# Medical-Image-Analysis-Laboratory/MSLesions3D

Hardware: AMD Instinct MI355X
Metric: training volumes/sec at 128^3 batch-4 (fwd+loss+bwd+Adam), data-parallel over N MI355X (higher is better)
Workload: dtype f32; 1 GPU; 128^3 synthetic volumes, batch 4/GPU, 1 channel(s), fp32, SSD3D+MobileNet3D full train step (BASELINE configs[1]); global_batch=4, parallelism=dp1, priors=9344

## Files before the change

### mslesions3d_amd/csrc/pwconv.hip

```cpp
#include "common.hpp"
#include <algorithm>
#include <cstdlib>

namespace {

typedef float f32x16 __attribute__((ext_vector_type(16)));

constexpr int BM = 64, BN = 128, BK = 32;
constexpr int FOLD_MAXK = 512;
constexpr int WS_LD = BK + 1;

template <bool AFFINE, bool STATS, bool TRANS_W>
__global__ __launch_bounds__(256) void pw_gemm_kernel(const float* __restrict__ X,
                                                      const float* __restrict__ in_scale,
                                                      const float* __restrict__ in_shift,
                                                      const float* __restrict__ Wt, float* __restrict__ Y,
                                                      double* __restrict__ partials, int M, int K, int S,
                                                      msl::BnFold fold) {
  __shared__ __align__(16) float Xs[BK][BN];
  __shared__ float Ws[BM][WS_LD];
  __shared__ float red[2][2][BM];
  __shared__ float f_sc[AFFINE ? FOLD_MAXK : 1], f_sh[AFFINE ? FOLD_MAXK : 1];
  const int n = blockIdx.z, m0 = blockIdx.y * BM, s0 = blockIdx.x * BN;
  const int tid = threadIdx.x, lane = tid & 63, wv = tid >> 6;
// ... 571 lines not shown
                     0, st, X, in_scale, in_shift, Wt, Y, partials, M, K, S, fold)
#define MSL_WV1(KW_, MT_)                                                                                              \
  do {                                                                                                                 \
    if (nt == 2)                                                                                                       \
      MSL_LAUNCH((pw_wave_kernel<KW_, MT_, AFFINE, STATS, TRANS_W, 1, 2>), dim3(msl::cdiv(S, 256), M / (32 * MT_), N), \
                         dim3(256), 0, st, X, in_scale, in_shift, Wt, Y, partials, M, K, S, fold);                     \
    else                                                                                                               \
      MSL_WV(KW_, MT_, 1);                                                                                             \
  } while (0)
  const bool two = M % 64 == 0;
  const int nt = STATS ? wave_nt(N, K, M, S) : 1;
  if (K == 32) {
    if (two) MSL_WV1(32, 2); else MSL_WV1(32, 1);
  } else if (K == 64) {
    if (two) MSL_WV1(64, 2); else MSL_WV1(64, 1);
  } else {
    switch (K / 64) {
      case 2: MSL_WV(64, 1, 2); break;
      case 4: MSL_WV(64, 1, 4); break;
      case 8: MSL_WV(64, 1, 8); break;
      default: return MSL_ERR_UNSUPPORTED;
    }
  }
#undef MSL_WV1
#undef MSL_WV
  MSL_LAUNCH_CHECK();
  return MSL_OK;
}

constexpr int PC = 64, PC_LD = PC + 1;

template <int BNN, bool AFFINE>
__global__ __launch_bounds__(256) void pw_bwd_weight_kernel(const float* __restrict__ dY,
                                                            const float* __restrict__ Z,
                                                            const float* __restrict__ in_scale,
                                                            const float* __restrict__ in_shift,
                                                            float* __restrict__ slabs, int Cout, int Cin,
                                                            int S, int N, int chunks_per_img,
                                                            int chunks_per_block) {
  constexpr int NSUB_N = BNN / 32;
  constexpr int NSUB = 2 * NSUB_N;
  __shared__ __align__(16) float lds[(64 + BNN) * PC_LD > 64 * BNN ? (64 + BNN) * PC_LD : 64 * BNN];
  float* dys = lds;
  float* as_ = lds + 64 * PC_LD;
  const int ks = blockIdx.x;
  const int tiles_n = Cin / BNN;
  const int tm = blockIdx.y / tiles_n, tn = blockIdx.y % tiles_n;
  const int m0 = tm * 64, n0 = tn * BNN;
  const int tid = threadIdx.x, lane = tid & 63, wv = tid >> 6;
  const int total_chunks = N * chunks_per_img;
  const int ch_lo = ks * chunks_per_block, ch_hi = min(total_chunks, ch_lo + chunks_per_block);
  const bool vec_ok = (S & 3) == 0;

  f32x16 acc[NSUB];
#pragma unroll
  for (int i = 0; i < NSUB; ++i) acc[i] = (f32x16){0};

  float scv[BNN / 16], shv[BNN / 16];
#pragma unroll
  for (int j = 0; j < BNN / 16; ++j) {
    scv[j] = AFFINE ? in_scale[n0 + (tid >> 4) + j * 16] : 1.f;
    shv[j] = AFFINE ? in_shift[n0 + (tid >> 4) + j * 16] : 0.f;
  }

  for (int ch = ch_lo; ch < ch_hi; ++ch) {
    const int n = ch / chunks_per_img, s0 = (ch % chunks_per_img) * PC;
    const float* dyn = dY + ((size_t)n * Cout + m0) * S;
    const float* zn = Z + ((size_t)n * Cin + n0) * S;
    float4 st[(64 + BNN) / 16];
    if (vec_ok) {
#pragma unroll
      for (int i = 0; i < (64 + BNN) / 16; ++i) {
        const int r = (tid >> 4) + i * 16;
        st[i] = msl::load4_zfill<true>(r < 64 ? dyn + (size_t)r * S : zn + (size_t)(r - 64) * S, s0 + (tid & 15) * 4, S);
      }
    } else {
#pragma unroll
      for (int i = 0; i < (64 + BNN) / 16; ++i) {
        const int r = (tid >> 4) + i * 16;
        st[i] = msl::load4_zfill<false>(r < 64 ? dyn + (size_t)r * S : zn + (size_t)(r - 64) * S, s0 + (tid & 15) * 4, S);
      }
    }
#pragma unroll
    for (int i = 0; i < (64 + BNN) / 16; ++i) {
      const int r = (tid >> 4) + i * 16, c4 = (tid & 15) * 4, col = s0 + c4;
      float4 v = st[i];
      if (AFFINE && r >= 64) {
        const float sc = scv[i >= 4 ? i - 4 : 0], sh = shv[i >= 4 ? i - 4 : 0];
        v.x = col < S ? msl::act(v.x, sc, sh) : 0.f;
        v.y = col + 1 < S ? msl::act(v.y, sc, sh) : 0.f;
        v.z = col + 2 < S ? msl::act(v.z, sc, sh) : 0.f;
        v.w = col + 3 < S ? msl::act(v.w, sc, sh) : 0.f;
      }
      float* dst = lds + r * PC_LD + c4;
      dst[0] = v.x; dst[1] = v.y; dst[2] = v.z; dst[3] = v.w;
    }
    __syncthreads();
#pragma unroll
    for (int kk = 0; kk < 8; ++kk) {
      const int pos = wv * 16 + 2 * kk + (lane >> 5);
      float a[2], b[NSUB_N];
#pragma unroll
      for (int i = 0; i < 2; ++i) a[i] = dys[(i * 32 + (lane & 31)) * PC_LD + pos];
#pragma unroll
      for (int j = 0; j < NSUB_N; ++j) b[j] = as_[(j * 32 + (lane & 31)) * PC_LD + pos];
#pragma unroll
      for (int i = 0; i < 2; ++i)
#pragma unroll
        for (int j = 0; j < NSUB_N; ++j)
          acc[i * NSUB_N + j] = __builtin_amdgcn_mfma_f32_32x32x2f32(a[i], b[j], acc[i * NSUB_N + j], 0, 0, 0);
    }
    __syncthreads();
  }

  float* redt = lds;
  for (int w = 3; w >= 1; --w) {
    if (wv == w) {
#pragma unroll
      for (int i = 0; i < 2; ++i)
#pragma unroll
        for (int j = 0; j < NSUB_N; ++j)
#pragma unroll
          for (int r = 0; r < 16; ++r) {
            const int row = i * 32 + (r & 3) + 8 * (r >> 2) + 4 * (lane >> 5);
            const int col = j * 32 + (lane & 31);
            const float v = acc[i * NSUB_N + j][r];
            if (w == 3) redt[row * BNN + col] = v;
            else redt[row * BNN + col] += v;
          }
    }
    __syncthreads();
  }
  if (wv == 0) {
    float* out = slabs + (size_t)ks * Cout * Cin;
#pragma unroll
    for (int i = 0; i < 2; ++i)
#pragma unroll
      for (int j = 0; j < NSUB_N; ++j)
#pragma unroll
        for (int r = 0; r < 16; ++r) {
          const int row = i * 32 + (r & 3) + 8 * (r >> 2) + 4 * (lane >> 5);
          const int col = j * 32 + (lane & 31);
          out[(size_t)(m0 + row) * Cin + n0 + col] = acc[i * NSUB_N + j][r] + redt[row * BNN + col];
        }
  }
}

template <int MT, bool AFFINE>
__device__ __forceinline__ void pw_bww_wave_body(const float* __restrict__ dY, const float* __restrict__ Z,
                                                 const float* __restrict__ in_scale, const float* __restrict__ in_shift,
                                                 float* __restrict__ out, int Cout, int Cin, int S, int chunks_per_img,
                                                 int total_chunks, int chunks_per_block, int ks, int tile) {
  __shared__ __align__(16) float red[4 * MT * 1024];
  const int lane = threadIdx.x & 63, wv = threadIdx.x >> 6, h = lane >> 5, c = lane & 31;
  const int tiles_n = Cin / 32;
  const int tm = tile / tiles_n, tn = tile % tiles_n;
  const int m0 = tm * 32 * MT, n0 = tn * 32;
  const int ch_lo = ks * chunks_per_block, ch_hi = min(total_chunks, ch_lo + chunks_per_block);
  const int mine = max(0, (ch_hi - ch_lo - wv + 3) / 4);

  float sc = 1.f, sh = 0.f;
  if (AFFINE) {
    sc = in_scale[n0 + c];
    sh = in_shift[n0 + c];
  }
  f32x16 acc[MT];
#pragma unroll
  for (int mt = 0; mt < MT; ++mt) acc[mt] = (f32x16){0};

  float4 a0[MT][4], b0[4], a1[MT][4], b1[4];
  auto issue = [&](int i, float4 (&a)[MT][4], float4 (&b)[4]) {
    const int ch = min(ch_lo + wv + 4 * i, total_chunks - 1);
    const int n = ch / chunks_per_img, s0 = (ch - n * chunks_per_img) * 32 + 16 * h;
#pragma unroll
    for (int mt = 0; mt < MT; ++mt) {
      const float4* p = reinterpret_cast<const float4*>(dY + ((size_t)n * Cout + m0 + mt * 32 + c) * S + s0);
#pragma unroll
      for (int j = 0; j < 4; ++j) a[mt][j] = p[j];
    }
    const float4* q = reinterpret_cast<const float4*>(Z + ((size_t)n * Cin + n0 + c) * S + s0);
#pragma unroll
    for (int j = 0; j < 4; ++j) b[j] = q[j];
  };
  auto mac = [&](float4 (&a)[MT][4], float4 (&b)[4]) {
#pragma unroll
    for (int j = 0; j < 4; ++j) {
      float bv[4] = {b[j].x, b[j].y, b[j].z, b[j].w};
#pragma unroll
      for (int e = 0; e < 4; ++e) {
        const float x = AFFINE ? msl::act(bv[e], sc, sh) : bv[e];
#pragma unroll
        for (int mt = 0; mt < MT; ++mt) {
          const float av = e == 0 ? a[mt][j].x : e == 1 ? a[mt][j].y : e == 2 ? a[mt][j].z : a[mt][j].w;
          acc[mt] = __builtin_amdgcn_mfma_f32_32x32x2f32(av, x, acc[mt], 0, 0, 0);
        }
      }
    }
  };

  if (mine > 0) issue(0, a0, b0);
#pragma unroll 1
  for (int i = 0; i < mine; i += 2) {
    issue(i + 1, a1, b1);
    __builtin_amdgcn_sched_barrier(0);
    mac(a0, b0);
    if (i + 1 < mine) {
      issue(i + 2, a0, b0);
      __builtin_amdgcn_sched_barrier(0);
      mac(a1, b1);
    }
  }

#pragma unroll
  for (int mt = 0; mt < MT; ++mt)
#pragma unroll
    for (int r = 0; r < 16; ++r) red[((wv * MT + mt) * 32 + (r & 3) + 8 * (r >> 2) + 4 * h) * 32 + c] = acc[mt][r];
  __syncthreads();
  float* dst = out + (size_t)ks * Cout * Cin;
#pragma unroll
  for (int e = 0; e < MT; ++e) {
    const int q4 = threadIdx.x + e * 256;
    const int row = q4 >> 3, col = (q4 & 7) * 4;
    float4 v = *reinterpret_cast<const float4*>(&red[(0 * MT * 32 + row) * 32 + col]);
#pragma unroll
    for (int w2 = 1; w2 < 4; ++w2) {
      const float4 t = *reinterpret_cast<const float4*>(&red[(w2 * MT * 32 + row) * 32 + col]);
      v.x += t.x; v.y += t.y; v.z += t.z; v.w += t.w;
    }
    *reinterpret_cast<float4*>(dst + (size_t)(m0 + row) * Cin + n0 + col) = v;
  }
}

template <int MT, bool AFFINE>
__global__ __launch_bounds__(256) void pw_bww_wave_kernel(const float* __restrict__ dY, const float* __restrict__ Z,
                                                          const float* __restrict__ in_scale,
                                                          const float* __restrict__ in_shift, float* __restrict__ out,
                                                          int Cout, int Cin, int S, int chunks_per_img, int total_chunks,
                                                          int chunks_per_block) {
  pw_bww_wave_body<MT, AFFINE>(dY, Z, in_scale, in_shift, out, Cout, Cin, S, chunks_per_img, total_chunks, chunks_per_block,
                               blockIdx.x, blockIdx.y);
}

constexpr int PW_BWW_BATCH_MAX = 4;
struct PwBwwBatch {
  const float* dY[PW_BWW_BATCH_MAX];
  const float* Z[PW_BWW_BATCH_MAX];
  const float* in_scale[PW_BWW_BATCH_MAX];
  const float* in_shift[PW_BWW_BATCH_MAX];
  float* out[PW_BWW_BATCH_MAX];
  int Cout[PW_BWW_BATCH_MAX], Cin[PW_BWW_BATCH_MAX], S[PW_BWW_BATCH_MAX], chunks_per_img[PW_BWW_BATCH_MAX],
      total_chunks[PW_BWW_BATCH_MAX], chunks_per_block[PW_BWW_BATCH_MAX], ksplit[PW_BWW_BATCH_MAX],
      first[PW_BWW_BATCH_MAX + 1];
};

__global__ __launch_bounds__(256) void pw_bww_wave_batch_kernel(PwBwwBatch b, int n) {
  int k = 0;
#pragma unroll
  for (int j = 1; j < PW_BWW_BATCH_MAX; ++j)
    if (j < n && (int)blockIdx.x >= b.first[j]) k = j;
  const int local = blockIdx.x - b.first[k];
  pw_bww_wave_body<2, true>(b.dY[k], b.Z[k], b.in_scale[k], b.in_shift[k], b.out[k], b.Cout[k], b.Cin[k], b.S[k],
                            b.chunks_per_img[k], b.total_chunks[k], b.chunks_per_block[k], local % b.ksplit[k],
                            local / b.ksplit[k]);
}

struct BwwWavePlan {
  int mt, tiles, chunks_per_img, total_chunks, ksplit, chunks_per_block;
};

static inline bool bww_wave_plan(int N, int Cin, int Cout, int S, BwwWavePlan& p) {
  constexpr int off = 1;
  if (!off || S % 32 != 0 || Cin % 32 != 0 || Cout % 32 != 0) return false;
  p.mt = (Cout % 64 == 0) ? 2 : 1;
  p.tiles = (Cout / (32 * p.mt)) * (Cin / 32);
  p.chunks_per_img = S / 32;
  p.total_chunks = N * p.chunks_per_img;
  constexpr int target = 256;
  int ks = std::max(1, std::min(target / std::max(1, p.tiles), p.total_chunks / 8));
  p.chunks_per_block = msl::cdiv(p.total_chunks, ks);
  p.ksplit = msl::cdiv(p.total_chunks, p.chunks_per_block);
  return true;
}

__global__ __launch_bounds__(256) void slab_reduce_kernel(const float* __restrict__ slabs, float* __restrict__ out,
                                                          int count, int nslabs) {
  __shared__ float lds[8 * 33];
  const float t = msl::reduce_slabs_256(slabs, (size_t)count, count, nslabs, lds);
  const int i = blockIdx.x * 32 + (threadIdx.x & 31);
  if ((threadIdx.x >> 5) == 0 && i < count) out[i] = t;
}

struct BwPlan {
  int bnn, ksplit, chunks_per_img, chunks_per_block;
};

BwPlan bw_plan(int N, int Cin, int Cout, int S) {
  BwPlan p;
  p.bnn = (Cin % 64 == 0) ? 64 : 32;
  p.chunks_per_img = msl::cdiv(S, PC);
  const int total = N * p.chunks_per_img;
  const int tiles = (Cout / 64) * (Cin / p.bnn);
  int ks = std::max(1, std::min(total, 512 / std::max(1, tiles)));
  constexpr int min_cpb = 1;
  ks = std::max(1, std::min(ks, total / std::max(1, min_cpb)));
  p.chunks_per_block = msl::cdiv(total, ks);
  p.ksplit = msl::cdiv(total, p.chunks_per_block);
  return p;
}

}

extern "C" {

static inline bool use_ksplit(int K, int M, int S, int N) {
  return K >= 128 && K % 128 == 0 && msl::cdiv(S, BN) * msl::cdiv(M, BM) * N < 256;
}

int msl_pwconv_fwd_num_partials(int N, int Cin, int Cout, int S) {
  if (const int cols = strip_cols(N, Cin, Cout, S)) return N * (S / cols);
  if (wave_form(Cin, Cout)) return N * msl::cdiv(S, Cin <= 64 ? 128 * wave_nt(N, Cin, Cout, S) : 32);
  return N * msl::cdiv(S, use_ksplit(Cin, Cout, S, N) ? KS_BN : BN);
}

static const msl::BnFold pw_nofold{nullptr, 0, 0, 1.0, nullptr, nullptr, 0.f};

static int pwconv_fwd_impl(const float* z, const float* in_scale, const float* in_shift, const msl::BnFold& fold,
                           const float* w, float* y, double* partials, int N, int Cin, int Cout, int S, void* stream) {
  if (N <= 0 || S <= 0 || Cin % BK != 0 || Cout % 4 != 0) return MSL_ERR_ARG;
  if ((in_scale || fold.partials) && Cin > FOLD_MAXK) return MSL_ERR_UNSUPPORTED;
  hipStream_t st = (hipStream_t)stream;
  if (const int cols = strip_cols(N, Cin, Cout, S)) {
    if (in_scale || fold.partials) {
      if (partials) return launch_strip<true, true, false>(z, in_scale, in_shift, w, y, partials, N, Cout, Cin, S, cols, fold, st);
      return launch_strip<true, false, false>(z, in_scale, in_shift, w, y, partials, N, Cout, Cin, S, cols, fold, st);
    }
    if (partials) return launch_strip<false, true, false>(z, in_scale, in_shift, w, y, partials, N, Cout, Cin, S, cols, fold, st);
    return launch_strip<false, false, false>(z, in_scale, in_shift, w, y, partials, N, Cout, Cin, S, cols, fold, st);
  }
  if (wave_form(Cin, Cout)) {
    if (in_scale || fold.partials) {
      if (partials) return launch_wave<true, true, false>(z, in_scale, in_shift, w, y, partials, N, Cout, Cin, S, fold, st);
      return launch_wave<true, false, false>(z, in_scale, in_shift, w, y, partials, N, Cout, Cin, S, fold, st);
    }
    if (partials) return launch_wave<false, true, false>(z, in_scale, in_shift, w, y, partials, N, Cout, Cin, S, fold, st);
    return launch_wave<false, false, false>(z, in_scale, in_shift, w, y, partials, N, Cout, Cin, S, fold, st);
  }
  if (use_ksplit(Cin, Cout, S, N)) {
    dim3 g2(msl::cdiv(S, KS_BN), msl::cdiv(Cout, KS_BM), N);
#define MSL_KS(A_, S_, T_, X_, Wp_, Y_, P_, M_, K_)                                                                  \
  do {                                                                                                             \
    if ((K_) % 256 == 0) {                                                                                         \
      const size_t lds_ = (size_t)8 * KS_WAVE_LDS * sizeof(float);                                                 \
      hipError_t e_ = hipFuncSetAttribute(reinterpret_cast<const void*>(pw_gemm_ksplit_kernel<A_, S_, T_, 8>),    \
                                          hipFuncAttributeMaxDynamicSharedMemorySize, (int)lds_);                  \
      if (e_ != hipSuccess) return (int)e_;                                                                        \
      MSL_LAUNCH((pw_gemm_ksplit_kernel<A_, S_, T_, 8>), g2, dim3(512), lds_, st, X_, in_scale, in_shift,  \
                         Wp_, Y_, P_, M_, K_, S, fold);                                                            \
    } else {                                                                                                       \
      MSL_LAUNCH((pw_gemm_ksplit_kernel<A_, S_, T_, 4>), g2, dim3(256),                                    \
                         (size_t)4 * KS_WAVE_LDS * sizeof(float), st, X_, in_scale, in_shift, Wp_, Y_, P_, M_, K_, S, fold); \
    }                                                                                                              \
  } while (0)
    if (in_scale || fold.partials) {
      if (partials) MSL_KS(true, true, false, z, w, y, partials, Cout, Cin);
      else MSL_KS(true, false, false, z, w, y, partials, Cout, Cin);
    } else {
      if (partials) MSL_KS(false, true, false, z, w, y, partials, Cout, Cin);
      else MSL_KS(false, false, false, z, w, y, partials, Cout, Cin);
    }
    MSL_LAUNCH_CHECK();
    return MSL_OK;
  }
  dim3 grid(msl::cdiv(S, BN), msl::cdiv(Cout, BM), N);
  if (in_scale || fold.partials) {
    if (partials) MSL_LAUNCH((pw_gemm_kernel<true, true, false>), grid, dim3(256), 0, st, z, in_scale, in_shift, w, y, partials, Cout, Cin, S, fold);
    else MSL_LAUNCH((pw_gemm_kernel<true, false, false>), grid, dim3(256), 0, st, z, in_scale, in_shift, w, y, partials, Cout, Cin, S, fold);
  } else {
    if (partials) MSL_LAUNCH((pw_gemm_kernel<false, true, false>), grid, dim3(256), 0, st, z, in_scale, in_shift, w, y, partials, Cout, Cin, S, fold);
    else MSL_LAUNCH((pw_gemm_kernel<false, false, false>), grid, dim3(256), 0, st, z, in_scale, in_shift, w, y, partials, Cout, Cin, S, fold);
  }
  MSL_LAUNCH_CHECK();
  return MSL_OK;
}

int msl_pwconv_fwd(const float* z, const float* in_scale, const float* in_shift, const float* w, float* y,
                   double* partials, int N, int Cin, int Cout, int S, void* stream) {
  return pwconv_fwd_impl(z, in_scale, in_shift, pw_nofold, w, y, partials, N, Cin, Cout, S, stream);
}

int msl_pwconv_fwd_fold(const float* z, const double* in_partials, int in_np, double in_count, const float* gamma,
                        const float* beta, float eps, const float* w, float* y, double* partials, int N, int Cin,
                        int Cout, int S, void* stream) {
  if (!in_partials || in_np <= 0) return MSL_ERR_ARG;
  const msl::BnFold fold{in_partials, in_np, Cin, in_count, gamma, beta, eps};
  return pwconv_fwd_impl(z, nullptr, nullptr, fold, w, y, partials, N, Cin, Cout, S, stream);
}

int msl_pwconv_bwd_data(const float* dy, const float* w, float* g_in, int N, int Cin, int Cout, int S,
                        void* stream) {
  if (N <= 0 || S <= 0 || Cout % BK != 0 || Cin % 4 != 0) return MSL_ERR_ARG;
  if (const int cols = strip_cols(N, Cout, Cin, S))
    return launch_strip<false, false, true>(dy, nullptr, nullptr, w, g_in, nullptr, N, Cin, Cout, S, cols, pw_nofold,
                                            (hipStream_t)stream);
  if (wave_form(Cout, Cin))
    return launch_wave<false, false, true>(dy, nullptr, nullptr, w, g_in, nullptr, N, Cin, Cout, S, pw_nofold,
                                           (hipStream_t)stream);
  if (use_ksplit(Cout, Cin, S, N)) {
    dim3 g2(msl::cdiv(S, KS_BN), msl::cdiv(Cin, KS_BM), N);
    hipStream_t st = (hipStream_t)stream;
    const float *in_scale = nullptr, *in_shift = nullptr;
    double* nopart = nullptr;
    const msl::BnFold fold = pw_nofold;
    MSL_KS(false, false, true, dy, w, g_in, nopart, Cin, Cout);
    MSL_LAUNCH_CHECK();
    return MSL_OK;
  }
  dim3 grid(msl::cdiv(S, BN), msl::cdiv(Cin, BM), N);
  MSL_LAUNCH((pw_gemm_kernel<false, false, true>), grid, dim3(256), 0, (hipStream_t)stream, dy, nullptr,
                     nullptr, w, g_in, nullptr, Cin, Cout, S, pw_nofold);
  MSL_LAUNCH_CHECK();
  return MSL_OK;
}

size_t msl_pwconv_bwd_weight_workspace_bytes(int N, int Cin, int Cout, int S) {
  BwwWavePlan wp;
  if (bww_wave_plan(N, Cin, Cout, S, wp)) return (size_t)wp.ksplit * Cout * Cin * sizeof(float);
  BwPlan p = bw_plan(N, Cin, Cout, S);
  return (size_t)p.ksplit * Cout * Cin * sizeof(float);
}

int msl_pwconv_bwd_weight_nslabs(int N, int Cin, int Cout, int S) {
// ... 85 lines not shown
```

### mslesions3d_amd/csrc/chanlink.hip

```cpp
#include "common.hpp"
#include "../../include/mslesions3d_hip.h"

namespace {

typedef float f32x4v __attribute__((ext_vector_type(4)));

template <typename T>
__device__ __forceinline__ f32x4v ldq(const T* p) {
  const float4 v = msl::ld4(p);
  return (f32x4v){v.x, v.y, v.z, v.w};
}
template <typename T>
__device__ __forceinline__ void stq(T* p, f32x4v v) { msl::st4(p, make_float4(v[0], v[1], v[2], v[3])); }
template <typename T>
__device__ __forceinline__ f32x4v rounded(const T* tag, f32x4v v) {
  const float4 r = msl::as_stored(tag, make_float4(v[0], v[1], v[2], v[3]));
  return (f32x4v){r.x, r.y, r.z, r.w};
}

template <int NW>
__device__ __forceinline__ void chan_sum2(double& a, double& b, double* scratch) {
  a = msl::wave_sum(a);
  b = msl::wave_sum(b);
  if (NW > 1) {
    const int lane = threadIdx.x & 63, w = threadIdx.x >> 6;
    __syncthreads();
    if (lane == 0) {
      scratch[2 * w] = a;
      scratch[2 * w + 1] = b;
    }
    __syncthreads();
    a = 0.0;
    b = 0.0;
#pragma unroll
    for (int i = 0; i < NW; ++i) {
      a += scratch[2 * i];
      b += scratch[2 * i + 1];
    }
  }
}

template <typename T, int NW, int QO, int QI, int STRIDE, bool BWW>
__global__ __launch_bounds__(NW * 64) void block_bwd_channel_link_kernel(
    T* __restrict__ g_z, const T* __restrict__ z, const float* __restrict__ vec_z, const float* __restrict__ w_dw,
    const T* __restrict__ y_prev, const float* __restrict__ vec_y, T* __restrict__ g_y,
    float* __restrict__ dgamma_z, float* __restrict__ dbeta_z, float* __restrict__ dgamma_y, float* __restrict__ dbeta_y,
    float* __restrict__ dw_dw, int N, int C, int lD, int lH, int lW, int accumulate) {
  constexpr int NT = NW * 64, LS = STRIDE == 2 ? 1 : 0;
  extern __shared__ __align__(16) float lds[];
  const int c = blockIdx.x, tid = threadIdx.x;
  const int lOD = lD - LS, lOH = lH - LS, lOW = lW - LS;
  const int OD = 1 << lOD, OH = 1 << lOH, OW = 1 << lOW;
  const int lSo = lOD + lOH + lOW, lSi = lD + lH + lW;
  const int tot_qo = N << (lSo - 2), tot_qi = N << (lSi - 2);
  const int PW = OW + 8, PP = (OH + 2) * PW, pimg = (OD + 2) * PP, ptot = N * pimg;
  double* scratch = reinterpret_cast<double*>(lds + (BWW ? max(ptot, 27 * NT + 27 * 4) : ptot));

  f32x4v gq[QO], zq[QO], yq[QI], aq[QI];
#pragma unroll
  for (int q = 0; q < QO; ++q) {
    const int qi = min(tid + q * NT, tot_qo - 1), n = qi >> (lSo - 2), r = qi & ((1 << (lSo - 2)) - 1);
    const size_t off = (((size_t)n * C + c) << lSo) + 4 * r;
    gq[q] = ldq(g_z + off);
    zq[q] = ldq(z + off);
  }
#pragma unroll
  for (int q = 0; q < QI; ++q) {
    const int qi = min(tid + q * NT, tot_qi - 1), n = qi >> (lSi - 2), r = qi & ((1 << (lSi - 2)) - 1);
    yq[q] = ldq(y_prev + (((size_t)n * C + c) << lSi) + 4 * r);
  }
  if (accumulate) {
#pragma unroll
    for (int q = 0; q < QI; ++q) {
      const int qi = min(tid + q * NT, tot_qi - 1), n = qi >> (lSi - 2), r = qi & ((1 << (lSi - 2)) - 1);
      aq[q] = ldq(g_y + (((size_t)n * C + c) << lSi) + 4 * r);
    }
  } else {
#pragma unroll
    for (int q = 0; q < QI; ++q) aq[q] = (f32x4v){0.f, 0.f, 0.f, 0.f};
  }
  const float sc1 = vec_z[c], sh1 = vec_z[C + c], mu1 = vec_z[2 * C + c], is1 = vec_z[3 * C + c];
  const float sc2 = vec_y[c], sh2 = vec_y[C + c], mu2 = vec_y[2 * C + c], is2 = vec_y[3 * C + c];
  float wt[27];
#pragma unroll
  for (int k = 0; k < 27; ++k) wt[k] = w_dw[c * 27 + k];
  for (int i = tid; i < (ptot >> 2); i += NT) reinterpret_cast<f32x4v*>(lds)[i] = (f32x4v){0.f, 0.f, 0.f, 0.f};

  float s1 = 0.f, s2 = 0.f;
#pragma unroll
  for (int q = 0; q < QO; ++q) {
    const bool in = tid + q * NT < tot_qo;
#pragma unroll
    for (int e = 0; e < 4; ++e) {
      const float gm = (in && fmaf(zq[q][e], sc1, sh1) > 0.f) ? gq[q][e] : 0.f;
      const float xh = (zq[q][e] - mu1) * is1;
      gq[q][e] = gm;
      zq[q][e] = xh;
      s1 += gm;
      s2 += gm * xh;
    }
  }
  double t1 = (double)s1, t2 = (double)s2;
  chan_sum2<NW>(t1, t2, scratch);
  {
    const double cnt_o = (double)(N << lSo);
    const float k1 = (float)(t1 / cnt_o), k2 = (float)(t2 / cnt_o);
    if (tid == 0) {
      dbeta_z[c] = (float)t1;
      dgamma_z[c] = (float)t2;
    }
    if (NW == 1) __syncthreads();
#pragma unroll
    for (int q = 0; q < QO; ++q) {
      const int qi = tid + q * NT;
      if (qi < tot_qo) {
        const int n = qi >> (lSo - 2), r = qi & ((1 << (lSo - 2)) - 1);
        f32x4v dz;
#pragma unroll
        for (int e = 0; e < 4; ++e) dz[e] = sc1 * (gq[q][e] - k1 - zq[q][e] * k2);
        stq(g_z + (((size_t)n * C + c) << lSo) + 4 * r, dz);
        dz = rounded(g_z, dz);
        const int s = 4 * r, ow = s & (OW - 1), oh = (s >> lOW) & (OH - 1), od = s >> (lOW + lOH);
        *reinterpret_cast<f32x4v*>(lds + n * pimg + (od + 1) * PP + (oh + 1) * PW + 4 + ow) = dz;
      }
    }
  }
  __syncthreads();

  s1 = 0.f;
  s2 = 0.f;
  const int W = 1 << lW, H = 1 << lH;
  float dwa[BWW ? 27 : 1];
#pragma unroll
  for (int k = 0; k < (BWW ? 27 : 1); ++k) dwa[k] = 0.f;
#pragma unroll
  for (int q = 0; q < QI; ++q) {
    const int qi = tid + q * NT;
    const bool in = qi < tot_qi;
    const int qc = in ? qi : 0, n = qc >> (lSi - 2), r = qc & ((1 << (lSi - 2)) - 1);
    const int s = 4 * r, iw = s & (W - 1), ih = (s >> lW) & (H - 1), id = s >> (lW + lH);
    f32x4v acc = aq[q];
    f32x4v av;
#pragma unroll
    for (int e = 0; e < 4; ++e) av[e] = (BWW && in) ? msl::act(yq[q][e], sc2, sh2) : 0.f;
    const float* img = lds + n * pimg + 4;
#pragma unroll
    for (int kd = 0; kd < 3; ++kd) {
      const int td = id + 1 - kd;
      if (STRIDE == 2 && (td & 1)) continue;
      const int pd = (STRIDE == 2 ? (td >> 1) : td) + 1;
#pragma unroll
      for (int kh = 0; kh < 3; ++kh) {
        const int th = ih + 1 - kh;
        if (STRIDE == 2 && (th & 1)) continue;
        const int ph = (STRIDE == 2 ? (th >> 1) : th) + 1;
        const float* row = img + pd * PP + ph * PW;
        const float w0 = wt[kd * 9 + kh * 3], w1 = wt[kd * 9 + kh * 3 + 1], w2 = wt[kd * 9 + kh * 3 + 2];
        if (STRIDE == 1) {
          const float lft = row[iw - 1], rgt = row[iw + 4];
          const f32x4v m = *reinterpret_cast<const f32x4v*>(row + iw);
          acc[0] = fmaf(w0, m[1], fmaf(w1, m[0], fmaf(w2, lft, acc[0])));
          acc[1] = fmaf(w0, m[2], fmaf(w1, m[1], fmaf(w2, m[0], acc[1])));
          acc[2] = fmaf(w0, m[3], fmaf(w1, m[2], fmaf(w2, m[1], acc[2])));
          acc[3] = fmaf(w0, rgt, fmaf(w1, m[3], fmaf(w2, m[2], acc[3])));
          if (BWW) {
            float& d0 = dwa[kd * 9 + kh * 3];
            float& d1 = dwa[kd * 9 + kh * 3 + 1];
            float& d2 = dwa[kd * 9 + kh * 3 + 2];
            d0 = fmaf(av[0], m[1], fmaf(av[1], m[2], fmaf(av[2], m[3], fmaf(av[3], rgt, d0))));
            d1 = fmaf(av[0], m[0], fmaf(av[1], m[1], fmaf(av[2], m[2], fmaf(av[3], m[3], d1))));
            d2 = fmaf(av[0], lft, fmaf(av[1], m[0], fmaf(av[2], m[1], fmaf(av[3], m[2], d2))));
          }
        } else {
          const int o = iw >> 1;
          const float2 r01 = *reinterpret_cast<const float2*>(row + o);
          const float r2 = row[o + 2];
          acc[0] = fmaf(w1, r01.x, acc[0]);
          acc[1] = fmaf(w0, r01.y, fmaf(w2, r01.x, acc[1]));
          acc[2] = fmaf(w1, r01.y, acc[2]);
          acc[3] = fmaf(w0, r2, fmaf(w2, r01.y, acc[3]));
          if (BWW) {
            float& d0 = dwa[kd * 9 + kh * 3];
            float& d1 = dwa[kd * 9 + kh * 3 + 1];
            float& d2 = dwa[kd * 9 + kh * 3 + 2];
            d0 = fmaf(av[1], r01.y, fmaf(av[3], r2, d0));
            d1 = fmaf(av[0], r01.x, fmaf(av[2], r01.y, d1));
            d2 = fmaf(av[1], r01.x, fmaf(av[3], r01.y, d2));
          }
        }
      }
    }
    acc = rounded(g_y, acc);
#pragma unroll
    for (int e = 0; e < 4; ++e) {
      const float gm = (in && fmaf(yq[q][e], sc2, sh2) > 0.f) ? acc[e] : 0.f;
      const float xh = (yq[q][e] - mu2) * is2;
      aq[q][e] = gm;
      yq[q][e] = xh;
      s1 += gm;
      s2 += gm * xh;
    }
  }
  if (BWW) {
    __syncthreads();
#pragma unroll
    for (int k = 0; k < 27; ++k) lds[k * NT + tid] = dwa[k];
    __syncthreads();
    constexpr int PART = NT / 4;
    for (int t = tid; t < 108; t += NT) {
      const int k = t >> 2, part = t & 3;
      const f32x4v* src = reinterpret_cast<const f32x4v*>(lds + k * NT + part * PART);
      double sum = 0.0;
#pragma unroll 4
      for (int i = 0; i < PART / 4; ++i) {
        const f32x4v v = src[i];
        sum += (double)v[0];
        sum += (double)v[1];
        sum += (double)v[2];
        sum += (double)v[3];
      }
      sum += msl::dpp_mov<0xB1>(sum);
      sum += msl::dpp_mov<0x4E>(sum);
      if (part == 0) dw_dw[c * 27 + k] = (float)sum;
    }
  }
  t1 = (double)s1;
  t2 = (double)s2;
  chan_sum2<NW>(t1, t2, scratch);
  const double cnt_i = (double)(N << lSi);
  const float k1 = (float)(t1 / cnt_i), k2 = (float)(t2 / cnt_i);
  if (tid == 0) {
    dbeta_y[c] = (float)t1;
    dgamma_y[c] = (float)t2;
  }
#pragma unroll
  for (int q = 0; q < QI; ++q) {
    const int qi = tid + q * NT;
    if (qi < tot_qi) {
      const int n = qi >> (lSi - 2), r = qi & ((1 << (lSi - 2)) - 1);
      f32x4v dy;
#pragma unroll
      for (int e = 0; e < 4; ++e) dy[e] = sc2 * (aq[q][e] - k1 - yq[q][e] * k2);
      stq(g_y + (((size_t)n * C + c) << lSi) + 4 * r, dy);
    }
  }
}

struct LinkPlan {
  int nw, qo, qi, lD, lH, lW;
  size_t smem;
};

static inline int ilog2_exact(int v) {
  int l = 0;
  while ((1 << l) < v) ++l;
  return (1 << l) == v ? l : -1;
}

bool link_plan(int N, int D, int H, int W, int stride, LinkPlan& p) {
  if (N <= 0 || D <= 0 || H <= 0 || W <= 0 || (stride != 1 && stride != 2)) return false;
  p.lD = ilog2_exact(D);
  p.lH = ilog2_exact(H);
  p.lW = ilog2_exact(W);
  if (p.lD < 0 || p.lH < 0 || p.lW < 2) return false;
  const int OD = (D - 1) / stride + 1, OH = (H - 1) / stride + 1, OW = (W - 1) / stride + 1;
  if (OW < 4 || (stride == 2 && (D < 2 || H < 2))) return false;
  const long long tqo = (long long)N * OD * OH * OW / 4, tqi = (long long)N * D * H * W / 4;
  if (tqi <= 128) p.nw = 1;
  else if (tqi <= 1024) p.nw = 4;
  else if (tqi <= 2048) p.nw = 8;
  else if (tqi <= 4096) p.nw = 16;
  else return false;
  const int nt = p.nw * 64;
  auto up = [](long long v) { return v <= 1 ? 1 : v <= 2 ? 2 : 4; };
  p.qi = up((tqi + nt - 1) / nt);
  p.qo = up((tqo + nt - 1) / nt);
  if (p.qo > 1) p.qo = p.qi;
  const size_t ptot = (size_t)N * (OD + 2) * (OH + 2) * (OW + 8);
  p.smem = std::max(ptot, (size_t)27 * nt + 27 * 4) * 4 + 2 * p.nw * sizeof(double);
  return p.smem <= 156 * 1024;
}

}

extern "C" int msl_block_bwd_channel_link_supported(int N, int D, int H, int W, int stride) {
  LinkPlan p;
  return link_plan(N, D, H, W, stride, p) ? p.nw : 0;
}

template <typename T>
static int link_launch(T* g_z, const T* z, const float* vec_z, const float* w_dw, const T* y_prev, const float* vec_y, T* g_y,
                       float* dgamma_z, float* dbeta_z, float* dgamma_y, float* dbeta_y, float* dw_dw, int N, int C, int D,
                       int H, int W, int stride, int accumulate, void* stream) {
  if (N <= 0 || C <= 0 || !g_z || !z || !vec_z || !w_dw || !y_prev || !vec_y || !g_y) return MSL_ERR_ARG;
  LinkPlan p;
  if (!link_plan(N, D, H, W, stride, p)) return MSL_ERR_UNSUPPORTED;
  hipStream_t st = (hipStream_t)stream;
#define MSL_LINK_B(NW_, QO_, QI_, S_, B_)                                                                                 \
  do {                                                                                                                   \
    auto k = block_bwd_channel_link_kernel<T, NW_, QO_, QI_, S_, B_>;                                                    \
    if (p.smem > 64 * 1024) (void)hipFuncSetAttribute((const void*)k, hipFuncAttributeMaxDynamicSharedMemorySize, (int)p.smem); \
    MSL_LAUNCH(k, dim3(C), dim3(NW_ * 64), p.smem, st, g_z, z, vec_z, w_dw, y_prev, vec_y, g_y, dgamma_z, dbeta_z, \
                       dgamma_y, dbeta_y, dw_dw, N, C, p.lD, p.lH, p.lW, accumulate);                                     \
  } while (0)
#define MSL_LINK_S(NW_, QO_, QI_, S_)                  \
  do {                                                 \
    if (dw_dw) MSL_LINK_B(NW_, QO_, QI_, S_, true);    \
    else MSL_LINK_B(NW_, QO_, QI_, S_, false);         \
  } while (0)
#define MSL_LINK_Q(NW_, S_)                                            \
  do {                                                                 \
    if (p.qi == 1) MSL_LINK_S(NW_, 1, 1, S_);                          \
    else if (p.qi == 2 && p.qo == 1) MSL_LINK_S(NW_, 1, 2, S_);        \
    else if (p.qi == 2) MSL_LINK_S(NW_, 2, 2, S_);                     \
    else if (p.qo == 1) MSL_LINK_S(NW_, 1, 4, S_);                     \
    else MSL_LINK_S(NW_, 4, 4, S_);                                    \
  } while (0)
#define MSL_LINK(NW_)                       \
  do {                                      \
    if (stride == 1) MSL_LINK_Q(NW_, 1);    \
    else MSL_LINK_Q(NW_, 2);                \
  } while (0)
  if (p.nw == 1) MSL_LINK(1);
  else if (p.nw == 4) MSL_LINK(4);
  else if (p.nw == 8) MSL_LINK(8);
  else MSL_LINK(16);
#undef MSL_LINK
#undef MSL_LINK_Q
#undef MSL_LINK_S
#undef MSL_LINK_B
  MSL_LAUNCH_CHECK();
  return MSL_OK;
}

extern "C" {

int msl_block_bwd_channel_link(float* g_z, const float* z, const float* vec_z, const float* w_dw, const float* y_prev,
                               const float* vec_y, float* g_y, float* dgamma_z, float* dbeta_z, float* dgamma_y,
                               float* dbeta_y, float* dw_dw, int N, int C, int D, int H, int W, int stride, int accumulate,
                               void* stream) {
  return link_launch<float>(g_z, z, vec_z, w_dw, y_prev, vec_y, g_y, dgamma_z, dbeta_z, dgamma_y, dbeta_y, dw_dw, N, C, D, H, W,
                            stride, accumulate, stream);
}

int msl_block_bwd_channel_link_bf16(void* g_z, const void* z, const float* vec_z, const float* w_dw, const void* y_prev,
                                    const float* vec_y, void* g_y, float* dgamma_z, float* dbeta_z, float* dgamma_y,
                                    float* dbeta_y, float* dw_dw, int N, int C, int D, int H, int W, int stride, int accumulate,
                                    void* stream) {
  return link_launch<msl::su16>((msl::su16*)g_z, (const msl::su16*)z, vec_z, w_dw, (const msl::su16*)y_prev, vec_y,
                                (msl::su16*)g_y, dgamma_z, dbeta_z, dgamma_y, dbeta_y, dw_dw, N, C, D, H, W, stride, accumulate,
                                stream);
}

}
```

Measured before the change: 6062 volumes/s.

## Issue all chunk loads up front for short wave loops and deepen k-split

In the weight-gradient wave kernel, when a wave owns at most four chunks, all dY and Z loads are now issued before any MFMA work. A compile-time-unrolled path handles these cases, so more loads are in flight at once than with the old two-stage ping-pong. The split heuristic now allows a deeper k-split (at least 4 chunks per block instead of 8), falling back to the old floor when the tile grid is small. The wave index is made scalar with readfirstlane. Costs are higher register pressure from four staged buffers and more partial slabs to reduce afterwards.

```diff
diff --git a/mslesions3d_amd/csrc/pwconv.hip b/mslesions3d_amd/csrc/pwconv.hip
--- a/mslesions3d_amd/csrc/pwconv.hip
+++ b/mslesions3d_amd/csrc/pwconv.hip
@@ -747,7 +747,8 @@
                                                  float* __restrict__ out, int Cout, int Cin, int S, int chunks_per_img,
                                                  int total_chunks, int chunks_per_block, int ks, int tile) {
   __shared__ __align__(16) float red[4 * MT * 1024];
-  const int lane = threadIdx.x & 63, wv = threadIdx.x >> 6, h = lane >> 5, c = lane & 31;
+  const int lane = threadIdx.x & 63, h = lane >> 5, c = lane & 31;
+  const int wv = __builtin_amdgcn_readfirstlane(threadIdx.x >> 6);
   const int tiles_n = Cin / 32;
   const int tm = tile / tiles_n, tn = tile % tiles_n;
   const int m0 = tm * 32 * MT, n0 = tn * 32;
@@ -763,7 +764,7 @@
 #pragma unroll
   for (int mt = 0; mt < MT; ++mt) acc[mt] = (f32x16){0};
 
-  float4 a0[MT][4], b0[4], a1[MT][4], b1[4];
+  float4 a[4][MT][4], b[4][4];
   auto issue = [&](int i, float4 (&a)[MT][4], float4 (&b)[4]) {
     const int ch = min(ch_lo + wv + 4 * i, total_chunks - 1);
     const int n = ch / chunks_per_img, s0 = (ch - n * chunks_per_img) * 32 + 16 * h;
@@ -793,16 +794,34 @@
     }
   };
 
-  if (mine > 0) issue(0, a0, b0);
+  if (mine <= 4) {
+    auto walk = [&](auto count) {
+      constexpr int NC = decltype(count)::value;
+#pragma unroll
+      for (int i = 0; i < NC; ++i) issue(i, a[i], b[i]);
+      __builtin_amdgcn_sched_barrier(0);
+#pragma unroll
+      for (int i = 0; i < NC; ++i) mac(a[i], b[i]);
+    };
+    switch (mine) {
+      case 1: walk(std::integral_constant<int, 1>{}); break;
+      case 2: walk(std::integral_constant<int, 2>{}); break;
+      case 3: walk(std::integral_constant<int, 3>{}); break;
+      case 4: walk(std::integral_constant<int, 4>{}); break;
+      default: break;
+    }
+  } else {
+    issue(0, a[0], b[0]);
 #pragma unroll 1
-  for (int i = 0; i < mine; i += 2) {
-    issue(i + 1, a1, b1);
-    __builtin_amdgcn_sched_barrier(0);
-    mac(a0, b0);
-    if (i + 1 < mine) {
-      issue(i + 2, a0, b0);
+    for (int i = 0; i < mine; i += 2) {
+      issue(i + 1, a[1], b[1]);
       __builtin_amdgcn_sched_barrier(0);
-      mac(a1, b1);
+      mac(a[0], b[0]);
+      if (i + 1 < mine) {
+        issue(i + 2, a[0], b[0]);
+        __builtin_amdgcn_sched_barrier(0);
+        mac(a[1], b[1]);
+      }
     }
   }
 
@@ -871,7 +890,9 @@
   p.chunks_per_img = S / 32;
   p.total_chunks = N * p.chunks_per_img;
   constexpr int target = 256;
-  int ks = std::max(1, std::min(target / std::max(1, p.tiles), p.total_chunks / 8));
+  auto split = [&](int floor) { return std::max(1, std::min(target / std::max(1, p.tiles), p.total_chunks / floor)); };
+  int ks = split(4);
+  if (p.tiles * ks < target / 2) ks = split(8);
   p.chunks_per_block = msl::cdiv(p.total_chunks, ks);
   p.ksplit = msl::cdiv(p.total_chunks, p.chunks_per_block);
   return true;
```

After: 6082 volumes/s, median of 5. About the same (+0.3%).

## Assign stride-2 channel-link input quads to threads by spatial parity class

Applied to the files above, without the earlier changes.

For the stride-2 transposed depthwise backward, input quads are now mapped to threads so that every wave shares one (depth, height) parity class, chosen wave-uniformly via readfirstlane. Each wave then runs only the 1, 2 or 4 kernel rows that contribute for its parity, with no per-tap parity branches and no divergence. This is meant to cut the branching and wasted work inside the unrolled 3x3 tap loop. In exchange it adds static constraints on NW/QI, forces QI=4 when NW=1 at stride 2, narrows the set of supported launch configurations (others now return unsupported), and reorders global loads and stores, which may hurt coalescing.

```diff
diff --git a/mslesions3d_amd/csrc/chanlink.hip b/mslesions3d_amd/csrc/chanlink.hip
--- a/mslesions3d_amd/csrc/chanlink.hip
+++ b/mslesions3d_amd/csrc/chanlink.hip
@@ -38,6 +38,35 @@
       b += scratch[2 * i + 1];
     }
   }
+}
+
+constexpr int ilog2c(int v) { return v <= 1 ? 0 : 1 + ilog2c(v >> 1); }
+
+template <int NW, int QI>
+__device__ __forceinline__ int link_parity_class(int q, int tid) {
+  constexpr int LNT = ilog2c(NW * 64);
+  static_assert(QI == 4 || (QI == 2 && NW >= 2) || (QI == 1 && NW >= 4), "the class bits must lie above the lane bits");
+  if (QI == 4) return q;
+  if (QI == 2) return 2 * q + __builtin_amdgcn_readfirstlane(tid >> (LNT - 1));
+  return __builtin_amdgcn_readfirstlane(tid >> (LNT - 2));
+}
+
+template <bool BWW, int KD, int KH>
+__device__ __forceinline__ f32x4v link_row_s2(const float* row, const float* wt, f32x4v av, f32x4v acc, float* dwa) {
+  constexpr int K = KD * 9 + KH * 3;
+  const float w0 = wt[K], w1 = wt[K + 1], w2 = wt[K + 2];
+  const float2 r01 = *reinterpret_cast<const float2*>(row);
+  const float r2 = row[2];
+  acc[0] = fmaf(w1, r01.x, acc[0]);
+  acc[1] = fmaf(w0, r01.y, fmaf(w2, r01.x, acc[1]));
+  acc[2] = fmaf(w1, r01.y, acc[2]);
+  acc[3] = fmaf(w0, r2, fmaf(w2, r01.y, acc[3]));
+  if (BWW) {
+    dwa[K] = fmaf(av[1], r01.y, fmaf(av[3], r2, dwa[K]));
+    dwa[K + 1] = fmaf(av[0], r01.x, fmaf(av[2], r01.y, dwa[K + 1]));
+    dwa[K + 2] = fmaf(av[1], r01.x, fmaf(av[3], r01.y, dwa[K + 2]));
+  }
+  return acc;
 }
 
 template <typename T, int NW, int QO, int QI, int STRIDE, bool BWW>
@@ -56,6 +85,24 @@
   const int PW = OW + 8, PP = (OH + 2) * PW, pimg = (OD + 2) * PP, ptot = N * pimg;
   double* scratch = reinterpret_cast<double*>(lds + (BWW ? max(ptot, 27 * NT + 27 * 4) : ptot));
 
+  auto in_quad = [&](int q, int& n, int& r) -> bool {
+    if constexpr (STRIDE == 1) {
+      const int qi = tid + q * NT, qc = min(qi, tot_qi - 1);
+      n = qc >> (lSi - 2);
+      r = qc & ((1 << (lSi - 2)) - 1);
+      return qi < tot_qi;
+    } else {
+      const int cls = link_parity_class<NW, QI>(q, tid), pa = cls >> 1, pb = (cls ^ pa) & 1;
+      const int rest = tid & ((NT * QI >> 2) - 1);
+      const int x = rest & ((1 << (lSi - 4)) - 1), nn = rest >> (lSi - 4);
+      const int iwq = x & ((1 << (lW - 2)) - 1), ih = ((x >> (lW - 2)) & ((1 << (lH - 1)) - 1)) * 2 + pb;
+      const int id = (x >> (lW + lH - 3)) * 2 + pa;
+      n = min(nn, N - 1);
+      r = (((id << lH) + ih) << (lW - 2)) + iwq;
+      return nn < N;
+    }
+  };
+
   f32x4v gq[QO], zq[QO], yq[QI], aq[QI];
 #pragma unroll
   for (int q = 0; q < QO; ++q) {
@@ -66,13 +113,15 @@
   }
 #pragma unroll
   for (int q = 0; q < QI; ++q) {
-    const int qi = min(tid + q * NT, tot_qi - 1), n = qi >> (lSi - 2), r = qi & ((1 << (lSi - 2)) - 1);
+    int n, r;
+    in_quad(q, n, r);
     yq[q] = ldq(y_prev + (((size_t)n * C + c) << lSi) + 4 * r);
   }
   if (accumulate) {
 #pragma unroll
     for (int q = 0; q < QI; ++q) {
-      const int qi = min(tid + q * NT, tot_qi - 1), n = qi >> (lSi - 2), r = qi & ((1 << (lSi - 2)) - 1);
+      int n, r;
+      in_quad(q, n, r);
       aq[q] = ldq(g_y + (((size_t)n * C + c) << lSi) + 4 * r);
     }
   } else {
@@ -129,34 +178,29 @@
 
   s1 = 0.f;
   s2 = 0.f;
-  const int W = 1 << lW, H = 1 << lH;
   float dwa[BWW ? 27 : 1];
 #pragma unroll
   for (int k = 0; k < (BWW ? 27 : 1); ++k) dwa[k] = 0.f;
 #pragma unroll
   for (int q = 0; q < QI; ++q) {
-    const int qi = tid + q * NT;
-    const bool in = qi < tot_qi;
-    const int qc = in ? qi : 0, n = qc >> (lSi - 2), r = qc & ((1 << (lSi - 2)) - 1);
-    const int s = 4 * r, iw = s & (W - 1), ih = (s >> lW) & (H - 1), id = s >> (lW + lH);
+    int n, r;
+    const bool in = in_quad(q, n, r);
+    const int iwq = r & ((1 << (lW - 2)) - 1), ih = (r >> (lW - 2)) & ((1 << lH) - 1), id = r >> (lW + lH - 2);
     f32x4v acc = aq[q];
     f32x4v av;
 #pragma unroll
     for (int e = 0; e < 4; ++e) av[e] = (BWW && in) ? msl::act(yq[q][e], sc2, sh2) : 0.f;
     const float* img = lds + n * pimg + 4;
-#pragma unroll
-    for (int kd = 0; kd < 3; ++kd) {
-      const int td = id + 1 - kd;
-      if (STRIDE == 2 && (td & 1)) continue;
-      const int pd = (STRIDE == 2 ? (td >> 1) : td) + 1;
-#pragma unroll
-      for (int kh = 0; kh < 3; ++kh) {
-        const int th = ih + 1 - kh;
-        if (STRIDE == 2 && (th & 1)) continue;
-        const int ph = (STRIDE == 2 ? (th >> 1) : th) + 1;
-        const float* row = img + pd * PP + ph * PW;
-        const float w0 = wt[kd * 9 + kh * 3], w1 = wt[kd * 9 + kh * 3 + 1], w2 = wt[kd * 9 + kh * 3 + 2];
-        if (STRIDE == 1) {
+    if constexpr (STRIDE == 1) {
+      const int iw = 4 * iwq;
+#pragma unroll
+      for (int kd = 0; kd < 3; ++kd) {
+        const int pd = id + 2 - kd;
+#pragma unroll
+        for (int kh = 0; kh < 3; ++kh) {
+          const int ph = ih + 2 - kh;
+          const float* row = img + pd * PP + ph * PW;
+          const float w0 = wt[kd * 9 + kh * 3], w1 = wt[kd * 9 + kh * 3 + 1], w2 = wt[kd * 9 + kh * 3 + 2];
           const float lft = row[iw - 1], rgt = row[iw + 4];
           const f32x4v m = *reinterpret_cast<const f32x4v*>(row + iw);
           acc[0] = fmaf(w0, m[1], fmaf(w1, m[0], fmaf(w2, lft, acc[0])));
@@ -171,23 +215,24 @@
             d1 = fmaf(av[0], m[0], fmaf(av[1], m[1], fmaf(av[2], m[2], fmaf(av[3], m[3], d1))));
             d2 = fmaf(av[0], lft, fmaf(av[1], m[0], fmaf(av[2], m[1], fmaf(av[3], m[2], d2))));
           }
-        } else {
-          const int o = iw >> 1;
-          const float2 r01 = *reinterpret_cast<const float2*>(row + o);
-          const float r2 = row[o + 2];
-          acc[0] = fmaf(w1, r01.x, acc[0]);
-          acc[1] = fmaf(w0, r01.y, fmaf(w2, r01.x, acc[1]));
-          acc[2] = fmaf(w1, r01.y, acc[2]);
-          acc[3] = fmaf(w0, r2, fmaf(w2, r01.y, acc[3]));
-          if (BWW) {
-            float& d0 = dwa[kd * 9 + kh * 3];
-            float& d1 = dwa[kd * 9 + kh * 3 + 1];
-            float& d2 = dwa[kd * 9 + kh * 3 + 2];
-            d0 = fmaf(av[1], r01.y, fmaf(av[3], r2, d0));
-            d1 = fmaf(av[0], r01.x, fmaf(av[2], r01.y, d1));
-            d2 = fmaf(av[1], r01.x, fmaf(av[3], r01.y, d2));
-          }
         }
+      }
+    } else {
+      const int cls = link_parity_class<NW, QI>(q, tid), pa = cls >> 1, pb = (cls ^ pa) & 1;
+      const float* row = img + ((id >> 1) + 1) * PP + ((ih >> 1) + 1) * PW + 2 * iwq;
+      if (pa == 0 && pb == 0) {
+        acc = link_row_s2<BWW, 1, 1>(row, wt, av, acc, dwa);
+      } else if (pa == 0) {
+        acc = link_row_s2<BWW, 1, 0>(row + PW, wt, av, acc, dwa);
+        acc = link_row_s2<BWW, 1, 2>(row, wt, av, acc, dwa);
+      } else if (pb == 0) {
+        acc = link_row_s2<BWW, 0, 1>(row + PP, wt, av, acc, dwa);
+        acc = link_row_s2<BWW, 2, 1>(row, wt, av, acc, dwa);
+      } else {
+        acc = link_row_s2<BWW, 0, 0>(row + PP + PW, wt, av, acc, dwa);
+        acc = link_row_s2<BWW, 0, 2>(row + PP, wt, av, acc, dwa);
+        acc = link_row_s2<BWW, 2, 0>(row + PW, wt, av, acc, dwa);
+        acc = link_row_s2<BWW, 2, 2>(row, wt, av, acc, dwa);
       }
     }
     acc = rounded(g_y, acc);
@@ -235,9 +280,8 @@
   }
 #pragma unroll
   for (int q = 0; q < QI; ++q) {
-    const int qi = tid + q * NT;
-    if (qi < tot_qi) {
-      const int n = qi >> (lSi - 2), r = qi & ((1 << (lSi - 2)) - 1);
+    int n, r;
+    if (in_quad(q, n, r)) {
       f32x4v dy;
 #pragma unroll
       for (int e = 0; e < 4; ++e) dy[e] = sc2 * (aq[q][e] - k1 - yq[q][e] * k2);
@@ -276,6 +320,7 @@
   p.qi = up((tqi + nt - 1) / nt);
   p.qo = up((tqo + nt - 1) / nt);
   if (p.qo > 1) p.qo = p.qi;
+  if (stride == 2 && p.nw == 1) p.qi = 4;
   const size_t ptot = (size_t)N * (OD + 2) * (OH + 2) * (OW + 8);
   p.smem = std::max(ptot, (size_t)27 * nt + 27 * 4) * 4 + 2 * p.nw * sizeof(double);
   return p.smem <= 156 * 1024;
@@ -308,25 +353,22 @@
     if (dw_dw) MSL_LINK_B(NW_, QO_, QI_, S_, true);    \
     else MSL_LINK_B(NW_, QO_, QI_, S_, false);         \
   } while (0)
-#define MSL_LINK_Q(NW_, S_)                                            \
-  do {                                                                 \
-    if (p.qi == 1) MSL_LINK_S(NW_, 1, 1, S_);                          \
-    else if (p.qi == 2 && p.qo == 1) MSL_LINK_S(NW_, 1, 2, S_);        \
-    else if (p.qi == 2) MSL_LINK_S(NW_, 2, 2, S_);                     \
-    else if (p.qo == 1) MSL_LINK_S(NW_, 1, 4, S_);                     \
-    else MSL_LINK_S(NW_, 4, 4, S_);                                    \
+  if (p.qo != (stride == 1 ? p.qi : 1)) return MSL_ERR_UNSUPPORTED;
+#define MSL_LINK(NW_, QI_)                              \
+  do {                                                  \
+    if (stride == 1) MSL_LINK_S(NW_, QI_, QI_, 1);      \
+    else MSL_LINK_S(NW_, 1, QI_, 2);                    \
   } while (0)
-#define MSL_LINK(NW_)                       \
-  do {                                      \
-    if (stride == 1) MSL_LINK_Q(NW_, 1);    \
-    else MSL_LINK_Q(NW_, 2);                \
-  } while (0)
-  if (p.nw == 1) MSL_LINK(1);
-  else if (p.nw == 4) MSL_LINK(4);
-  else if (p.nw == 8) MSL_LINK(8);
-  else MSL_LINK(16);
+  if (p.nw == 1 && stride == 2 && p.qi == 4) MSL_LINK_S(1, 1, 4, 2);
+  else if (p.nw == 1 && stride == 1 && p.qi == 1) MSL_LINK_S(1, 1, 1, 1);
+  else if (p.nw == 1 && stride == 1 && p.qi == 2) MSL_LINK_S(1, 2, 2, 1);
+  else if (p.nw == 4 && p.qi == 1) MSL_LINK(4, 1);
+  else if (p.nw == 4 && p.qi == 2) MSL_LINK(4, 2);
+  else if (p.nw == 4 && p.qi == 4) MSL_LINK(4, 4);
+  else if (p.nw == 8 && p.qi == 4) MSL_LINK(8, 4);
+  else if (p.nw == 16 && p.qi == 4) MSL_LINK(16, 4);
+  else return MSL_ERR_UNSUPPORTED;
 #undef MSL_LINK
-#undef MSL_LINK_Q
 #undef MSL_LINK_S
 #undef MSL_LINK_B
   MSL_LAUNCH_CHECK();
```

New measurement: 6073 volumes/s before, 6156 volumes/s after (median of 6 runs). 1.4% higher.
